# schwallergroup/matinvent

Measured on AMD Instinct MI355X. Metric: crystal structures/sec (1000-step reverse diffusion), higher is better.
Workload: dtype f32 via 2-plane fp16 split (3 fp16 MFMA terms, f32 accumulate)

## Files before the change

### matinvent_amd/csrc/edge_stage.hip

```cpp
#include <mutex>

#include <cstdio>
#include <cstdlib>
#include "net.h"
#include "gemm_split.h"
#define MI_LOOP_BARRIER() __builtin_amdgcn_s_barrier()
#define MI_RING_WAIT(w) asm volatile("s_waitcnt vmcnt(20)" : "+v"((w)[0][0]), "+v"((w)[0][1]), "+v"((w)[1][0]), "+v"((w)[1][1]))

namespace mi {

extern int g_edge2_train;
int g_edge2_fused = 1;

#if MI_PLANES_FP16

struct EdgeGemm2Args {
    Planes A;
    const u16* W2f;
    const float* b2;
    const float* dsc;
    const int* src;
    const int* rowptr;
    float* part;
    int E, N;
    const int* tab = nullptr;
    float* Z2 = nullptr;
    unsigned long long* clk;
};

constexpr int EG2_TAB = 2 + 128 + 128;
__global__ __launch_bounds__(128) void edge2_tables_kernel(const int* __restrict__ src, const int* __restrict__ rowptr, int E, int N, int* __restrict__ tab) {
    const int tile = blockIdx.x, tid = threadIdx.x, row0 = tile * 128;
    if (row0 >= E) return;
    const int nrows = E - row0 < 128 ? E - row0 : 128;
    const int node_first = src[row0];
    int* t = tab + (size_t)tile * EG2_TAB;
    const int r = row0 + tid, node = node_first + tid;
    t[2 + tid] = r < E ? src[r] - node_first : -1;
    t[130 + tid] = node < N ? tile - (rowptr[node] >> 7) : 0;
    if (tid == 0) {
        t[0] = node_first;
        t[1] = src[row0 + nrows - 1] - node_first + 1;
    }
}

constexpr int EG2B_STAGE = 2 * 128 * 64, EG2B_NST = 4;
constexpr int EG2B_LDS = EG2B_NST * EG2B_STAGE + 128 * 4 + 128 * 4;

template <int D, bool SAVE_Z = false>
__global__ __launch_bounds__(256) __attribute__((amdgpu_waves_per_eu(2, 2))) void edge_gemm2b_kernel(EdgeGemm2Args a) {
    constexpr int H = 512, KS = H / 16, KT = H / 32;
    extern __shared__ __attribute__((aligned(16))) unsigned char smem[];
    int* srcl = reinterpret_cast<int*>(smem + EG2B_NST * EG2B_STAGE);
    int* slotb = srcl + 128;
    const int tid = threadIdx.x, lane = tid & 63, wave = __builtin_amdgcn_readfirstlane(tid >> 6);
    const int l31 = lane & 31, kg = lane >> 5;
    const int id = blockIdx.x, slot = id >> 3, half = slot & 1, tile = (slot >> 1) * 8 + (id & 7);
    const int row0 = tile * 128;
    if (row0 >= a.E) return;
    const int nrows = a.E - row0 < 128 ? a.E - row0 : 128;
    int stamp_i = 0;
    auto stamp = [&]() {
        if (a.clk && tid == 0) a.clk[(size_t)(tile * 2 + half) * 8 + stamp_i] = __builtin_amdgcn_s_memtime();
        ++stamp_i;
    };
    stamp();
    if (a.clk && tid == 0) a.clk[(size_t)(tile * 2 + half) * 8 + 4] = __builtin_amdgcn_s_memrealtime();

    const int* tab = a.tab + (size_t)tile * EG2_TAB;
    int t_srcl = -1, t_slotb = 0;
    if (tid < 128) {
        t_srcl = tab[2 + tid];
        t_slotb = tab[130 + tid];
    }
    const int node_first = tab[0], cnt_tab = tab[1];

    const __amdgpu_buffer_rsrc_t rsa = uniform_rsrc(a.A.base + a.A.tile(tile, 0), a.A.KT * 24576);
    const int voffa = (lane >> 2) * 64 + (((lane & 3) ^ ((lane >> 4) & 3)) << 4);
    auto dma_tile = [&](int kt, int st) {
#pragma unroll
        for (int q = 0; q < 4; ++q) {
            const int piece = wave * 4 + q;
            __builtin_amdgcn_raw_ptr_buffer_load_lds(rsa, (__attribute__((address_space(3))) void*)(smem + st * EG2B_STAGE + piece * 1024), 16, voffa,
                                                     kt * 24576 + (piece >> 3) * 8192 + (piece & 7) * 1024, 0, 0);
        }
    };
    dma_tile(0, 0);
    dma_tile(1, 1);
    dma_tile(2, 2);

    int voffw[2];
#pragma unroll
    for (int t = 0; t < 2; ++t) voffw[t] = lane * 16 + ((8 * half + 2 * wave + t) * KS) * 2048;
    u32x4 ring[D][2][2];
    const u32x4 rsw_s = rsrc_words(a.W2f, H * H * 4);
    auto ring_load = [&](int ks, u32x4 (&w)[2][2]) {
        const int soff = __builtin_amdgcn_readfirstlane(ks * 2048);
#pragma unroll
        for (int t = 0; t < 2; ++t) {
            asm volatile("buffer_load_dwordx4 %0, %1, %2, %3 offen" : "=v"(w[t][0]) : "v"(voffw[t]), "s"(rsw_s), "s"(soff));
            asm volatile("buffer_load_dwordx4 %0, %1, %2, %3 offen offset:1024" : "=v"(w[t][1]) : "v"(voffw[t]), "s"(rsw_s), "s"(soff));
        }
    };
#pragma unroll
    for (int d = 0; d < D; ++d) ring_load(d, ring[d]);

    if (tid < 128) {
        srcl[tid] = t_srcl;
        slotb[tid] = t_slotb;
    }
    const float os = a.dsc[1] * (1.f / PL_SW), s_m2 = a.dsc[2], inv_m2 = a.dsc[3];

    f32x16 acc[4][2];
#pragma unroll
    for (int i = 0; i < 4; ++i)
#pragma unroll
        for (int j = 0; j < 2; ++j)
#pragma unroll
            for (int r = 0; r < 16; ++r) acc[i][j][r] = 0.f;
    const unsigned lds0 = (unsigned)(uintptr_t)(__attribute__((address_space(3))) unsigned char*)smem;
    unsigned rd_off[2];
#pragma unroll
    for (int s2 = 0; s2 < 2; ++s2) rd_off[s2] = lds0 + (unsigned)(l31 * 64 + (((2 * s2 + kg) ^ ((l31 >> 2) & 3)) * 16));
    auto read_a = [&](int st, int s2, f16x8 (&af)[4][2]) {
        const unsigned va = rd_off[s2] + (unsigned)st * EG2B_STAGE;
#define MI_RD128(dst, off) asm volatile("ds_read_b128 %0, %1 offset:%2" : "=v"(dst) : "v"(va), "n"(off))
        MI_RD128(af[0][0], 0 * 2048);        MI_RD128(af[0][1], 0 * 2048 + 8192);
        MI_RD128(af[1][0], 1 * 2048);        MI_RD128(af[1][1], 1 * 2048 + 8192);
        MI_RD128(af[2][0], 2 * 2048);        MI_RD128(af[2][1], 2 * 2048 + 8192);
        MI_RD128(af[3][0], 3 * 2048);        MI_RD128(af[3][1], 3 * 2048 + 8192);
#undef MI_RD128
    };
    auto mma = [&](const u32x4 (&w)[2][2], f16x8 (&af)[4][2]) {
#pragma unroll
        for (int ip = 0; ip < 2; ++ip) {
            if (ip == 0) asm volatile("s_waitcnt lgkmcnt(4)" : "+v"(af[0][0]), "+v"(af[0][1]), "+v"(af[1][0]), "+v"(af[1][1]));
            else asm volatile("s_waitcnt lgkmcnt(0)" : "+v"(af[2][0]), "+v"(af[2][1]), "+v"(af[3][0]), "+v"(af[3][1]));
#pragma unroll
            for (int term = MI_TERM0; term < 3; ++term)
#pragma unroll
                for (int i = 2 * ip; i < 2 * ip + 2; ++i)
#pragma unroll
                    for (int j = 0; j < 2; ++j)
                        acc[i][j] = __builtin_amdgcn_mfma_f32_32x32x16_f16(af[i][term == 0 ? 1 : 0], __builtin_bit_cast(f16x8, w[j][term == 1 ? 1 : 0]), acc[i][j], 0, 0, 0);
        }
    };
    static_assert(D == 4, "two k-tiles of ring per unrolled pair of iterations");
#pragma unroll 1
    for (int kt = 0; kt < KT; kt += 2) {
#pragma unroll
        for (int h2 = 0; h2 < 2; ++h2) {
            const int k = kt + h2;
            if (k == 0 || k >= KT - 3) asm volatile("s_waitcnt vmcnt(0)" ::: "memory");
            else asm volatile("s_waitcnt vmcnt(24)" ::: "memory");
            MI_LOOP_BARRIER();
            if (k == 0) stamp();
            if (k + 3 < KT) dma_tile(k + 3, (k + 3) & 3);
            f16x8 af[4][2];
#pragma unroll
            for (int s2 = 0; s2 < 2; ++s2) {
                read_a(k & 3, s2, af);
                MI_RING_WAIT(ring[2 * h2 + s2]);
                mma(ring[2 * h2 + s2], af);
                if (2 * k + s2 + D < KS) ring_load(2 * k + s2 + D, ring[2 * h2 + s2]);
                __builtin_amdgcn_sched_barrier(0);
            }
        }
    }
    stamp();

    if constexpr (SAVE_Z) {
        __syncthreads();
        float* stage = reinterpret_cast<float*>(smem) + wave * 1152;
#pragma unroll
        for (int i = 0; i < 4; ++i)
#pragma unroll
            for (int j = 0; j < 2; ++j) {
                const int rb = row0 + i * 32, cb = half * 256 + wave * 64 + j * 32;
#pragma unroll
                for (int r = 0; r < 16; ++r) stage[((r & 3) + 8 * (r >> 2) + 4 * kg) * 36 + l31] = acc[i][j][r] * os;
                __builtin_amdgcn_wave_barrier();
#pragma unroll
                for (int u = 0; u < 2; ++u) {
                    const int q = lane + 64 * u, rl = q >> 2, c8 = (q & 3) * 8;
                    const int row = rb + rl, col = cb + c8;
                    f32x4 z0 = *reinterpret_cast<const f32x4*>(stage + rl * 36 + c8);
                    f32x4 z1 = *reinterpret_cast<const f32x4*>(stage + rl * 36 + c8 + 4);
                    if (row < a.E) {
                        z0 += *reinterpret_cast<const f32x4*>(a.b2 + col);
                        z1 += *reinterpret_cast<const f32x4*>(a.b2 + col + 4);
                        float* d = a.Z2 + (size_t)row * H + col;
                        *reinterpret_cast<f32x4*>(d) = z0;
                        *reinterpret_cast<f32x4*>(d + 4) = z1;
                    }
                }
                __builtin_amdgcn_wave_barrier();
            }
    }

    const int cnt = nrows > 0 ? cnt_tab : 0;
    u16* sfr = reinterpret_cast<u16*>(smem);
    unsigned sat = 0;
    const int nlb = (cnt + 31) >> 5;
    __syncthreads();
    for (int f = tid; f < nlb * 8 * 64; f += 256) {
        const int ln = f & 63, fu = (f >> 6) & 1, frb = (f >> 7) & 3, fq = f >> 9;
        const int me = fq * 32 + (ln & 31), fkg = ln >> 5;
        u32x4 w;
#pragma unroll
        for (int i2 = 0; i2 < 4; ++i2) {
            const int ia = 2 * i2, ib = 2 * i2 + 1;
            const int ra = frb * 32 + 4 * fkg + 8 * (2 * fu + (ia >> 2)) + (ia & 3), rbb = frb * 32 + 4 * fkg + 8 * (2 * fu + (ib >> 2)) + (ib & 3);
            w[i2] = (srcl[ra] == me ? 0x3C00u : 0u) | (srcl[rbb] == me ? 0x3C000000u : 0u);
        }
        *reinterpret_cast<u32x4*>(sfr + (size_t)f * 8) = w;
    }
    __syncthreads();
#pragma unroll
    for (int j = 0; j < 2; ++j) {
        __builtin_amdgcn_sched_barrier(0);
        const int col = half * 256 + wave * 64 + j * 32 + l31;
        const float bcol = a.b2[col];
#pragma unroll 1
        for (int lb0 = 0; lb0 < nlb; lb0 += 2) {
            const bool two = lb0 + 1 < nlb;
            f32x16 ps[2];
#pragma unroll
            for (int q = 0; q < 2; ++q)
#pragma unroll
                for (int r = 0; r < 16; ++r) ps[q][r] = 0.f;
#pragma unroll
            for (int rb = 0; rb < 4; ++rb) {
                const f32x16 av = acc[rb][j];
#pragma unroll
                for (int u = 0; u < 2; ++u) {
                    f16x8 mh, ml;
#pragma unroll
                    for (int idx = 0; idx < 8; idx += 2) {
                        const float v0 = silu_fast(av[8 * u + idx] * os + bcol), v1 = silu_fast(av[8 * u + idx + 1] * os + bcol);
                        unsigned p[3];
                        pl_split_pair_acc(v0, v1, s_m2, p, sat);
                        const f16x2 h = __builtin_bit_cast(f16x2, p[0]), lo = __builtin_bit_cast(f16x2, p[1]);
                        mh[idx] = h[0]; mh[idx + 1] = h[1];
                        ml[idx] = lo[0]; ml[idx + 1] = lo[1];
                    }
#pragma unroll
                    for (int q = 0; q < 2; ++q) {
                        if (q == 1 && !two) break;
                        const f16x8 sf = *reinterpret_cast<const f16x8*>(sfr + (size_t)((((lb0 + q) * 4 + rb) * 2 + u) * 64 + lane) * 8);
                        ps[q] = __builtin_amdgcn_mfma_f32_32x32x16_f16(sf, ml, ps[q], 0, 0, 0);
                        ps[q] = __builtin_amdgcn_mfma_f32_32x32x16_f16(sf, mh, ps[q], 0, 0, 0);
                    }
                    __builtin_amdgcn_sched_barrier(0);
                }
            }
#pragma unroll
            for (int q = 0; q < 2; ++q)
#pragma unroll
                for (int r = 0; r < 16; ++r) {
                    const int loc = (lb0 + q) * 32 + (r & 3) + 8 * (r >> 2) + 4 * kg;
                    if (loc < cnt) a.part[((size_t)slotb[loc] * a.N + node_first + loc) * H + col] = ps[q][r] * inv_m2;
                }
        }
    }
    stamp();
    if (a.clk && tid == 0) a.clk[(size_t)(tile * 2 + half) * 8 + 5] = __builtin_amdgcn_s_memrealtime();
    sat_report(sat);
}

template <bool EXT, bool LEAN = false>
__global__ __launch_bounds__(256) __attribute__((amdgpu_waves_per_eu(2, 2))) void gemm_rt_kernel(Planes A, const u16* __restrict__ Wf, int M, int N, int K,
                                                                                                 PlanesEpilogue pe, unsigned long long* __restrict__ clk) {
    const int KS = K >> 4, KT = K >> 5;
    extern __shared__ __attribute__((aligned(16))) unsigned char smem[];
    M = pe.rows(M);
    const int tid = threadIdx.x, lane = tid & 63, wave = __builtin_amdgcn_readfirstlane(tid >> 6);
    int stamp_i = 0;
    auto stamp = [&]() {
        if (clk && tid == 0) clk[(size_t)blockIdx.x * 8 + stamp_i] = __builtin_amdgcn_s_memtime();
        ++stamp_i;
    };
    stamp();
    if (clk && tid == 0) clk[(size_t)blockIdx.x * 8 + 4] = __builtin_amdgcn_s_memrealtime();
    const int l31 = lane & 31, kg = lane >> 5;
    const int ncb = N >> 8;
    const int id = blockIdx.x, slot = id >> 3, cb = slot % ncb, tile = (slot / ncb) * 8 + (id & 7);
    const int row0 = tile * 128;
    if (row0 >= M) return;

    const __amdgpu_buffer_rsrc_t rsa = uniform_rsrc(A.base + A.tile(tile, 0), A.KT * 24576);
    const int voffa = (lane >> 2) * 64 + (((lane & 3) ^ ((lane >> 4) & 3)) << 4);
    auto dma_tile = [&](int kt, int st) {
#pragma unroll
        for (int q = 0; q < 4; ++q) {
            const int piece = wave * 4 + q;
            __builtin_amdgcn_raw_ptr_buffer_load_lds(rsa, (__attribute__((address_space(3))) void*)(smem + st * EG2B_STAGE + piece * 1024), 16, voffa,
                                                     kt * 24576 + (piece >> 3) * 8192 + (piece & 7) * 1024, 0, 0);
        }
    };
    dma_tile(0, 0);
    dma_tile(1, 1);
    dma_tile(2, 2);

    int voffw[2];
#pragma unroll
    for (int t = 0; t < 2; ++t) voffw[t] = lane * 16 + ((8 * cb + 2 * wave + t) * KS) * 2048;
    u32x4 ring[4][2][2];
    const u32x4 rsw_s = rsrc_words(Wf, N * K * 4);
    auto ring_load = [&](int ks, u32x4 (&w)[2][2]) {
        const int soff = __builtin_amdgcn_readfirstlane(ks * 2048);
#pragma unroll
        for (int t = 0; t < 2; ++t) {
            asm volatile("buffer_load_dwordx4 %0, %1, %2, %3 offen" : "=v"(w[t][0]) : "v"(voffw[t]), "s"(rsw_s), "s"(soff));
            asm volatile("buffer_load_dwordx4 %0, %1, %2, %3 offen offset:1024" : "=v"(w[t][1]) : "v"(voffw[t]), "s"(rsw_s), "s"(soff));
        }
    };
#pragma unroll
    for (int d = 0; d < 4; ++d) ring_load(d, ring[d]);

    f32x16 acc[4][2];
#pragma unroll
    for (int i = 0; i < 4; ++i)
#pragma unroll
        for (int j = 0; j < 2; ++j)
#pragma unroll
            for (int r = 0; r < 16; ++r) acc[i][j][r] = 0.f;
    const unsigned lds0 = (unsigned)(uintptr_t)(__attribute__((address_space(3))) unsigned char*)smem;
    unsigned rd_off[2];
#pragma unroll
    for (int s2 = 0; s2 < 2; ++s2) rd_off[s2] = lds0 + (unsigned)(l31 * 64 + (((2 * s2 + kg) ^ ((l31 >> 2) & 3)) * 16));
    auto read_a = [&](int st, int s2, f16x8 (&af)[4][2]) {
        const unsigned va = rd_off[s2] + (unsigned)st * EG2B_STAGE;
#define MI_RD128(dst, off) asm volatile("ds_read_b128 %0, %1 offset:%2" : "=v"(dst) : "v"(va), "n"(off))
        MI_RD128(af[0][0], 0 * 2048);        MI_RD128(af[0][1], 0 * 2048 + 8192);
        MI_RD128(af[1][0], 1 * 2048);        MI_RD128(af[1][1], 1 * 2048 + 8192);
        MI_RD128(af[2][0], 2 * 2048);        MI_RD128(af[2][1], 2 * 2048 + 8192);
        MI_RD128(af[3][0], 3 * 2048);        MI_RD128(af[3][1], 3 * 2048 + 8192);
#undef MI_RD128
    };
    auto mma = [&](const u32x4 (&w)[2][2], f16x8 (&af)[4][2]) {
#pragma unroll
        for (int ip = 0; ip < 2; ++ip) {
            if (ip == 0) asm volatile("s_waitcnt lgkmcnt(4)" : "+v"(af[0][0]), "+v"(af[0][1]), "+v"(af[1][0]), "+v"(af[1][1]));
            else asm volatile("s_waitcnt lgkmcnt(0)" : "+v"(af[2][0]), "+v"(af[2][1]), "+v"(af[3][0]), "+v"(af[3][1]));
#pragma unroll
            for (int term = MI_TERM0; term < 3; ++term)
#pragma unroll
                for (int i = 2 * ip; i < 2 * ip + 2; ++i)
#pragma unroll
                    for (int j = 0; j < 2; ++j)
                        if constexpr (LEAN)
                            acc[i][j] = __builtin_amdgcn_mfma_f32_32x32x16_f16(__builtin_bit_cast(f16x8, w[j][term == 1 ? 1 : 0]), af[i][term == 0 ? 1 : 0], acc[i][j], 0, 0, 0);
                        else
                            acc[i][j] = __builtin_amdgcn_mfma_f32_32x32x16_f16(af[i][term == 0 ? 1 : 0], __builtin_bit_cast(f16x8, w[j][term == 1 ? 1 : 0]), acc[i][j], 0, 0, 0);
        }
    };
#pragma unroll 1
    for (int kt = 0; kt < KT; kt += 2) {
#pragma unroll
        for (int h2 = 0; h2 < 2; ++h2) {
            const int k = kt + h2;
            if (k == 0 || k >= KT - 3) asm volatile("s_waitcnt vmcnt(0)" ::: "memory");
            else asm volatile("s_waitcnt vmcnt(24)" ::: "memory");
            MI_LOOP_BARRIER();
            if (k == 0) stamp();
            if (k + 3 < KT) dma_tile(k + 3, (k + 3) & 3);
            f16x8 af[4][2];
#pragma unroll
            for (int s2 = 0; s2 < 2; ++s2) {
                read_a(k & 3, s2, af);
                MI_RING_WAIT(ring[2 * h2 + s2]);
                mma(ring[2 * h2 + s2], af);
                if (2 * k + s2 + 4 < KS) ring_load(2 * k + s2 + 4, ring[2 * h2 + s2]);
                __builtin_amdgcn_sched_barrier(0);
            }
        }
    }
    __syncthreads();
    stamp();
    if constexpr (LEAN) planes_epilogue_lean<4, 2>(pe, acc, tile, cb * 256 + wave * 64, M, lane);
    else planes_epilogue_rows<4, 2, EXT>(pe, acc, row0, cb * 256 + wave * 64, M, N, lane, reinterpret_cast<float*>(smem) + wave * 1152);
    stamp();
    if (clk && tid == 0) clk[(size_t)blockIdx.x * 8 + 5] = __builtin_amdgcn_s_memrealtime();
}

__global__ void pack_frag_from_planes_kernel(Planes W, int N, int K, u16* __restrict__ dst) {
    const int KS = K / 16;
    const int64_t idx = (int64_t)blockIdx.x * blockDim.x + threadIdx.x;
    if (idx >= (int64_t)N * (K / 8)) return;
    const int r = (int)(idx / (K / 8)), ch = (int)(idx % (K / 8));
    const int ct = r >> 5, l31 = r & 31, ks = ch >> 1, kg = ch & 1;
#pragma unroll
    for (int pl = 0; pl < 2; ++pl)
        *reinterpret_cast<u32x4*>(dst + ((((size_t)ct * KS + ks) * 2 + pl) * 64 + kg * 32 + l31) * 8) = *reinterpret_cast<const u32x4*>(W.base + W.elem(r, ch * 8, pl));
}

int g_edge1_fused = 9;

__global__ void pack_frag_wff_pair_kernel(const float* __restrict__ W1, int edge_in, int H, int F, int Kh, u16* __restrict__ dst) {
    const int K = 2 * Kh, KS = K / 16, F3 = 3 * F;
    const int64_t idx = (int64_t)blockIdx.x * blockDim.x + threadIdx.x;
    if (idx >= (int64_t)H * (K / 8)) return;
    const int r = (int)(idx / (K / 8)), ch = (int)(idx % (K / 8));
    const int ct = r >> 5, l31 = r & 31, ks = ch >> 1, kg = ch & 1;
    float v[8];
#pragma unroll
    for (int i = 0; i < 8; ++i) {
        const int c = ch * 8 + i, blk = c >= Kh, cc = blk ? c - Kh : c;
        v[i] = cc < F3 ? W1[(size_t)r * edge_in + 2 * H + 9 + blk * F3 + cc] : 0.f;
    }
    u32x4 pk[2];
#pragma unroll
    for (int i = 0; i < 4; ++i) {
        unsigned p[3];
        pl_split_pair(v[2 * i], v[2 * i + 1], PL_SW, p);
        pk[0][i] = p[0];
        pk[1][i] = p[1];
    }
#pragma unroll
    for (int pl = 0; pl < 2; ++pl) *reinterpret_cast<u32x4*>(dst + ((((size_t)ct * KS + ks) * 2 + pl) * 64 + kg * 32 + l31) * 8) = pk[pl];
}

template <int D, bool WIDE>
__device__ __forceinline__ void edge_gemm1_body(const Planes& A, const u16* __restrict__ Wf, int M, int N, int K, PlanesEpilogue& pe, unsigned long long* clk) {
    extern __shared__ __attribute__((aligned(16))) unsigned char smem[];
    const int tid = threadIdx.x, lane = tid & 63, wave = __builtin_amdgcn_readfirstlane(tid >> 6);
    const int l31 = lane & 31, kg = lane >> 5;
    constexpr int MI = 4, NJ = 1;
    constexpr int WM = 4 / MI, WN = 4 / WM, WGC = 32 * NJ * WN;
    const int KT = K / 32, KS = K / 16, nq = N / WGC;
    const int wm = wave / WN, wn = wave % WN;
    const int id = blockIdx.x;
    float cps_local = 0.f;
    auto eval_scales = [&]() {
        if (pe.sc_pq) {
            float dsc[6];
            act_scales_eval(__uint_as_float(pe.sc_pq[0]), __uint_as_float(pe.sc_gmax[0]), pe.sc_wb, dsc);
            cps_local = dsc[0];
            if (id == 0 && tid < 6) {
                pe.sc_dsc[tid] = dsc[tid];
                if (pe.sc_dsc2) pe.sc_dsc2[tid] = dsc[tid];
            }
        }
    };
    eval_scales();
    if (pe.diag_C0 && id >= pe.diag_block0) {
        const float cps = cps_local != 0.f ? cps_local : pe.Cp.s();
        const int n0 = (id - pe.diag_block0) * 8, n1 = n0 + 8 < pe.diag_nodes ? n0 + 8 : pe.diag_nodes;
        const float* PQ = pe.ep.row_bias;
        const int ldpq = pe.ep.ld_row_bias;
        for (int f = 2 * tid; f < N; f += 512) {
            const float c0 = pe.diag_C0[f], c1 = pe.diag_C0[f + 1];
            for (int i = n0; i < n1; ++i) {
                const int e = pe.diag_e[i], g = pe.diag_node2graph[i];
                const float* G = pe.ep.row_bias3 + (size_t)g * pe.ep.ld_row_bias3;
                const float v0 = c0 + ((PQ[(size_t)i * ldpq + f] + PQ[(size_t)i * ldpq + N + f]) + G[f]);
                const float v1 = c1 + ((PQ[(size_t)i * ldpq + f + 1] + PQ[(size_t)i * ldpq + N + f + 1]) + G[f + 1]);
                if (pe.ep.pre_act) {
                    pe.ep.pre_act[(size_t)e * pe.ep.ld_pre + f] = v0;
                    pe.ep.pre_act[(size_t)e * pe.ep.ld_pre + f + 1] = v1;
                }
                unsigned p[3];
                pl_split_pair(silu_fast(v0), silu_fast(v1), cps, p);
#pragma unroll
                for (int k = 0; k < NPL; ++k) *reinterpret_cast<unsigned*>(pe.Cp.base + pe.Cp.elem(e, f, k)) = p[k];
            }
        }
        return;
    }
    const int slot = id >> 3, qt = slot % nq, tile = (slot / nq) * 8 + (id & 7);
    const int row0 = tile * 128;
    if (row0 >= M) return;
    int stamp_i = 0;
    auto stamp = [&]() {
        if (clk && tid == 0) clk[(size_t)(tile * nq + qt) * 8 + stamp_i] = __builtin_amdgcn_s_memtime();
        ++stamp_i;
    };
    stamp();

    const __amdgpu_buffer_rsrc_t rsa = uniform_rsrc(A.base + A.tile(tile, 0), A.KT * 24576);
    const int voffa = (lane >> 2) * 64 + (((lane & 3) ^ ((lane >> 4) & 3)) << 4);
    auto dma_tile = [&](int kt, int st) {
#pragma unroll
        for (int q = 0; q < 4; ++q) {
            const int piece = wave * 4 + q;
            __builtin_amdgcn_raw_ptr_buffer_load_lds(rsa, (__attribute__((address_space(3))) void*)(smem + st * EG2B_STAGE + piece * 1024), 16, voffa,
                                                     kt * 24576 + (piece >> 3) * 8192 + (piece & 7) * 1024, 0, 0);
        }
    };
    dma_tile(0, 0);
    dma_tile(1, 1);
    dma_tile(2, 2);
    const __amdgpu_buffer_rsrc_t rsw = uniform_rsrc(Wf, N * K * 4);
    int voffw[NJ];
#pragma unroll
    for (int t = 0; t < NJ; ++t) voffw[t] = lane * 16 + (((WN * qt + wn) * NJ + t) * KS) * 2048;
    u32x4 ring[D][NJ][2];
    const u32x4 rsw_s = rsrc_words(Wf, N * K * 4);
    auto ring_load = [&](int ks, u32x4 (&w)[NJ][2]) {
        const int soff = __builtin_amdgcn_readfirstlane(ks * 2048);
        asm volatile("buffer_load_dwordx4 %0, %1, %2, %3 offen" : "=v"(w[0][0]) : "v"(voffw[0]), "s"(rsw_s), "s"(soff));
        asm volatile("buffer_load_dwordx4 %0, %1, %2, %3 offen offset:1024" : "=v"(w[0][1]) : "v"(voffw[0]), "s"(rsw_s), "s"(soff));
    };
#pragma unroll
    for (int d = 0; d < D; ++d) ring_load(d, ring[d]);

    f32x16 acc[MI][NJ], accS[MI][NJ];
#pragma unroll
    for (int i = 0; i < MI; ++i)
#pragma unroll
        for (int j = 0; j < NJ; ++j)
#pragma unroll
            for (int r = 0; r < 16; ++r) acc[i][j][r] = 0.f;
    const unsigned lds0 = (unsigned)(uintptr_t)(__attribute__((address_space(3))) unsigned char*)smem;
    unsigned rd_off[2];
#pragma unroll
    for (int s2 = 0; s2 < 2; ++s2) rd_off[s2] = lds0 + (unsigned)(l31 * 64 + (((2 * s2 + kg) ^ ((l31 >> 2) & 3)) * 16));
    auto read_a = [&](int st, int s2, f16x8 (&af)[MI][2]) {
        const unsigned va = rd_off[s2] + (unsigned)st * EG2B_STAGE;
#define MI_RD128(dst, off) asm volatile("ds_read_b128 %0, %1 offset:%2" : "=v"(dst) : "v"(va), "n"(off))
        MI_RD128(af[0][0], 0 * 2048);        MI_RD128(af[0][1], 0 * 2048 + 8192);
        MI_RD128(af[1][0], 1 * 2048);        MI_RD128(af[1][1], 1 * 2048 + 8192);
        MI_RD128(af[2][0], 2 * 2048);        MI_RD128(af[2][1], 2 * 2048 + 8192);
        MI_RD128(af[3][0], 3 * 2048);        MI_RD128(af[3][1], 3 * 2048 + 8192);
#undef MI_RD128
    };
    auto mma = [&](u32x4 (&w)[NJ][2], f16x8 (&af)[MI][2]) {
        asm volatile("s_waitcnt vmcnt(14)" : "+v"(w[0][0]), "+v"(w[0][1]));
#pragma unroll
        for (int ip = 0; ip < 2; ++ip) {
            if (ip == 0) asm volatile("s_waitcnt lgkmcnt(4)" : "+v"(af[0][0]), "+v"(af[0][1]), "+v"(af[1][0]), "+v"(af[1][1]));
            else asm volatile("s_waitcnt lgkmcnt(0)" : "+v"(af[2][0]), "+v"(af[2][1]), "+v"(af[3][0]), "+v"(af[3][1]));
#pragma unroll
            for (int term = MI_TERM0; term < 3; ++term)
#pragma unroll
                for (int i = 2 * ip; i < 2 * ip + 2; ++i)
                    acc[i][0] = __builtin_amdgcn_mfma_f32_32x32x16_f16(af[i][term == 0 ? 1 : 0], __builtin_bit_cast(f16x8, w[0][term == 1 ? 1 : 0]), acc[i][0], 0, 0, 0);
        }
    };
    static_assert(D == 4, "two k-tiles of ring per unrolled pair of iterations");
    const int khalf = KT / 2;
#pragma unroll 1
    for (int kt = 0; kt < KT; kt += 2) {
#pragma unroll
        for (int h2 = 0; h2 < 2; ++h2) {
            const int k = kt + h2;
            if (k == khalf) {
#pragma unroll
                for (int i = 0; i < MI; ++i)
#pragma unroll
                    for (int j = 0; j < NJ; ++j) {
                        accS[i][j] = acc[i][j];
#pragma unroll
                        for (int r = 0; r < 16; ++r) acc[i][j][r] = 0.f;
                    }
            }
            if (k == 0 || k >= KT - 3) asm volatile("s_waitcnt vmcnt(0)" ::: "memory");
            else asm volatile("s_waitcnt vmcnt(16)" ::: "memory");
            MI_LOOP_BARRIER();
            if (k == 0) stamp();
            if (k + 3 < KT) dma_tile(k + 3, (k + 3) & 3);
            f16x8 af[MI][2];
#pragma unroll
            for (int s2 = 0; s2 < 2; ++s2) {
                read_a(k & 3, s2, af);
                mma(ring[2 * h2 + s2], af);
                if (2 * k + s2 + D < KS) ring_load(2 * k + s2 + D, ring[2 * h2 + s2]);
                __builtin_amdgcn_sched_barrier(0);
            }
        }
    }
    stamp();
    __syncthreads();
    planes_epilogue_pairs<MI, NJ, WIDE>(pe, accS, acc, row0 + wm * MI * 32, qt * WGC + wn * 32 * NJ, M, N, lane, reinterpret_cast<float*>(smem) + wave * 2304, cps_local);
    stamp();
}

template <int D, bool WIDE = true>
__global__ __launch_bounds__(256) __attribute__((amdgpu_waves_per_eu(2, 2))) void edge_gemm1b_kernel(Planes A, const u16* __restrict__ Wf, int M, int N, int K,
                                                                                                     PlanesEpilogue pe, unsigned long long* clk) {
    edge_gemm1_body<D, WIDE>(A, Wf, M, N, K, pe, clk);
}

unsigned long long* g_edge1_clk = nullptr;

__global__ void empty_boundary_kernel() {}

int edge_gemm1(mi_net* net, const Planes& A, int layer, int M, PlanesEpilogue pe, hipStream_t s) {
    if (g_ablate_skip & 2) return MI_OK;
    if (g_ablate_skip & 32) hipLaunchKernelGGL(empty_boundary_kernel, dim3(1), dim3(64), 0, s);
    static std::once_flag once;
    static hipError_t attr_err = hipSuccess;
    std::call_once(once, [] {
        attr_err = hipFuncSetAttribute((const void*)edge_gemm1b_kernel<4>, hipFuncAttributeMaxDynamicSharedMemorySize, EG2B_LDS);
        if (attr_err == hipSuccess) attr_err = hipFuncSetAttribute((const void*)edge_gemm1b_kernel<4, false>, hipFuncAttributeMaxDynamicSharedMemorySize, EG2B_LDS);
    });
    MI_HIP(attr_err);
    const int H = net->H, K = 2 * net->Kh;
    count_mfma(M, H, K, MI_PLANES_TERMS);
    pe.out_scale = 1.f / (A.scale * PL_SW);
    int nblk = (H / 128) * ((cdiv(M, 128) + 7) / 8 * 8);
    if (pe.diag_C0) {
        pe.diag_block0 = nblk;
        nblk += cdiv(pe.diag_nodes, 8);
    }
    const u16* Wf = net->Wffc + (size_t)layer * ((size_t)H * K * 2);
    if (pe.pair_wide) hipLaunchKernelGGL((edge_gemm1b_kernel<4>), dim3(nblk), dim3(256), EG2B_LDS, s, A, Wf, M, H, K, pe, g_edge1_clk);
    else hipLaunchKernelGGL((edge_gemm1b_kernel<4, false>), dim3(nblk), dim3(256), EG2B_LDS, s, A, Wf, M, H, K, pe, g_edge1_clk);
    MI_KERNEL_CHECK();
    return MI_OK;
}

bool edge_gemm1_supported(const mi_net* net, int64_t M) {
    if (!(net->H % 128 == 0 && net->Wffc != nullptr && (2 * net->Kh) % 64 == 0) || g_edge1_fused == 0) return false;
    if (g_edge1_fused != 9) return true;
    return (int64_t)(net->H / 128) * ((cdiv(M, 128) + 7) / 8 * 8) > g_planes_lat_max_blocks;
}

int edge_gemm1_pack(mi_net* net, int l, const float* W1, hipStream_t s) {
    const int H = net->H, K = 2 * net->Kh;
    hipLaunchKernelGGL(pack_frag_wff_pair_kernel, dim3(cdiv((int64_t)H * (K / 8), 256)), dim3(256), 0, s, W1, net->edge_in, H, net->F, net->Kh,
                       net->Wffc + (size_t)l * ((size_t)H * K * 2));
    MI_KERNEL_CHECK();
    return MI_OK;
}

unsigned long long* g_edge2_clk = nullptr;

int edge_gemm2(mi_net* net, mi_batch* b, int layer, hipStream_t s, float* Z2) {
    if (g_ablate_skip & 4) return MI_OK;
    if (g_ablate_skip & 32) hipLaunchKernelGGL(empty_boundary_kernel, dim3(1), dim3(64), 0, s);
    static std::once_flag once;
    static hipError_t attr_err = hipSuccess;
    std::call_once(once, [] {
        attr_err = hipFuncSetAttribute((const void*)edge_gemm2b_kernel<4>, hipFuncAttributeMaxDynamicSharedMemorySize, EG2B_LDS);
        if (attr_err == hipSuccess) attr_err = hipFuncSetAttribute((const void*)edge_gemm2b_kernel<4, true>, hipFuncAttributeMaxDynamicSharedMemorySize, EG2B_LDS);
    });
    MI_HIP(attr_err);
    const int H = net->H;
    count_mfma(b->E, H, H, MI_PLANES_TERMS);
    EdgeGemm2Args a;
    a.A = make_planes(b->m1_cur ? b->m1_cur : b->M1pl, H, PL_S_ACT, b->dsc);
    a.W2f = net->Wnc + (size_t)layer * node_chain_pack_elems(H) + (size_t)5 * H * H * 2;
    a.b2 = net->p("csp_layer_" + std::to_string(layer) + ".edge_mlp.2.bias");
    a.dsc = b->dsc;
    a.src = b->src;
    a.rowptr = b->rowptr;
    a.part = b->part;
    a.E = (int)b->E;
    a.N = b->N;
    {
        const int tiles_cap = cdiv(b->E_cap, 128);
        if (!b->e2_tab) MI_TRY(dev_alloc(b, &b->e2_tab, (size_t)tiles_cap * EG2_TAB));
        if (b->e2_tab_epoch != b->graph_epoch) {
            hipLaunchKernelGGL(edge2_tables_kernel, dim3(cdiv(b->E, 128)), dim3(128), 0, s, b->src, b->rowptr, (int)b->E, b->N, b->e2_tab);
            MI_KERNEL_CHECK();
            b->e2_tab_epoch = b->graph_epoch;
        }
        a.tab = b->e2_tab;
    }
    a.Z2 = Z2;
    a.clk = g_edge2_clk;
    if (Z2) {
        hipLaunchKernelGGL((edge_gemm2b_kernel<4, true>), dim3(2 * ((cdiv(b->E, 128) + 7) / 8 * 8)), dim3(256), EG2B_LDS, s, a);
        MI_KERNEL_CHECK();
        return MI_OK;
    }
    hipLaunchKernelGGL((edge_gemm2b_kernel<4>), dim3(2 * ((cdiv(b->E, 128) + 7) / 8 * 8)), dim3(256), EG2B_LDS, s, a);
    MI_KERNEL_CHECK();
    return MI_OK;
}

bool edge_gemm2_supported(const mi_net* net) { return g_edge2_fused && net->H == 512 && net->Wnc != nullptr; }

unsigned long long* g_rt_clk = nullptr;
int g_rt_clk_ext = -1;
int g_rt_lean = 1;
int g_rt_clk_skip = 0;

int gemm_rt(const Planes& A, const u16* Wfrag, int M, int N, int K, const PlanesEpilogue& pe, bool ext, hipStream_t s) {
    static std::once_flag once;
    static hipError_t attr_err = hipSuccess;
    std::call_once(once, [] {
        attr_err = hipFuncSetAttribute((const void*)gemm_rt_kernel<false>, hipFuncAttributeMaxDynamicSharedMemorySize, EG2B_NST * EG2B_STAGE);
        if (attr_err == hipSuccess) attr_err = hipFuncSetAttribute((const void*)gemm_rt_kernel<true>, hipFuncAttributeMaxDynamicSharedMemorySize, EG2B_NST * EG2B_STAGE);
        if (attr_err == hipSuccess) attr_err = hipFuncSetAttribute((const void*)gemm_rt_kernel<false, true>, hipFuncAttributeMaxDynamicSharedMemorySize, EG2B_NST * EG2B_STAGE);
        if (const char* e = getenv("MI_RT_LEAN")) g_rt_lean = atoi(e) & 3;
    });
    MI_HIP(attr_err);
    MI_CHECK(Wfrag && (N & 255) == 0 && (K & 63) == 0 && K >= 128 && A.KT >= K / 32, MI_EINVAL, "gemm_rt: N % 256, K % 64, K >= 128 and a fragment-order W operand");
    if (M <= 0) return MI_OK;
    count_mfma(M, N, K, MI_PLANES_TERMS);
    const dim3 grid((N >> 8) * ((cdiv(M, 128) + 7) / 8 * 8));
    static const bool trace = getenv("MI_RT_TRACE") != nullptr;
    if (trace)
        fprintf(stderr, "gemm_rt M=%d N=%d K=%d ext=%d act=%d bias=%d rb=%d%d%d pre_add=%d pre_act=%d res=%d res_pl=%d os=%g res2=%d res2_pl=%d rows2=%d post_mul=%d C=%d Cp=%d absmax=%d\n", M, N, K,
                (int)ext, pe.ep.act, !!pe.ep.bias, !!pe.ep.row_bias, !!pe.ep.row_bias2, !!pe.ep.row_bias3, !!pe.ep.pre_add, !!pe.ep.pre_act, !!pe.ep.residual, !!pe.res_pl.base,
                (double)pe.ep.out_scale, !!pe.residual2, !!pe.res2_pl.base, !!pe.res2_rows, !!pe.post_mul, !!pe.C, !!pe.Cp.base, !!pe.absmax);
    unsigned long long* clk = nullptr;
    if (g_rt_clk && (g_rt_clk_ext < 0 || g_rt_clk_ext == (int)ext)) {
        if (g_rt_clk_skip > 0) {
            --g_rt_clk_skip;
        } else {
            clk = g_rt_clk;
            if (g_rt_clk_ext >= 0) g_rt_clk = nullptr;
        }
    }
    if (g_rt_lean && planes_epilogue_is_lean(pe)) hipLaunchKernelGGL((gemm_rt_kernel<false, true>), grid, dim3(256), EG2B_NST * EG2B_STAGE, s, A, Wfrag, M, N, K, pe, clk);
    else if (ext) hipLaunchKernelGGL(gemm_rt_kernel<true>, grid, dim3(256), EG2B_NST * EG2B_STAGE, s, A, Wfrag, M, N, K, pe, clk);
    else hipLaunchKernelGGL(gemm_rt_kernel<false>, grid, dim3(256), EG2B_NST * EG2B_STAGE, s, A, Wfrag, M, N, K, pe, clk);
    MI_KERNEL_CHECK();
    return MI_OK;
}

size_t frag_elems(int N, int K) { return (size_t)N * K * 2; }

int pack_frag_from_planes(const Planes& W, int N, int K, u16* dst, hipStream_t s) {
    MI_CHECK((N & 31) == 0 && (K & 15) == 0, MI_EINVAL, "pack_frag_from_planes: N % 32, K % 16");
    hipLaunchKernelGGL(pack_frag_from_planes_kernel, dim3((unsigned)cdiv((int64_t)N * (K / 8), 256)), dim3(256), 0, s, W, N, K, dst);
    MI_KERNEL_CHECK();
    return MI_OK;
}

#else

int gemm_rt(const Planes&, const u16*, int, int, int, const PlanesEpilogue&, bool, hipStream_t) { return MI_ESTATE; }
size_t frag_elems(int N, int K) { return (size_t)N * K * 2; }
int pack_frag_from_planes(const Planes&, int, int, u16*, hipStream_t) { return MI_ESTATE; }

int edge_gemm2(mi_net*, mi_batch*, int, hipStream_t, float*) { return MI_ESTATE; }
bool edge_gemm2_supported(const mi_net*) { return false; }
int edge_gemm1(mi_net*, const Planes&, int, int, PlanesEpilogue, hipStream_t) { return MI_ESTATE; }
bool edge_gemm1_supported(const mi_net*, int64_t) { return false; }
int edge_gemm1_pack(mi_net*, int, const float*, hipStream_t) { return MI_OK; }
int g_edge1_fused = 0;

#endif

}

extern "C" int mi_debug_set_rt_lean(int on) {
#if MI_PLANES_FP16
    const int was = mi::g_rt_lean;
    mi::g_rt_lean = on & 3;
    return was;
#else
    (void)on;
    return 0;
#endif
}

extern "C" int mi_debug_rt_clock(void* dev_buffer, int ext, int skip) {
#if MI_PLANES_FP16
    mi::g_rt_clk = (unsigned long long*)dev_buffer;
    mi::g_rt_clk_ext = ext;
    mi::g_rt_clk_skip = skip;
#else
    (void)dev_buffer; (void)ext; (void)skip;
#endif
    return MI_OK;
}

extern "C" int mi_debug_edge2_clock(void* dev_buffer) {
#if MI_PLANES_FP16
    mi::g_edge2_clk = (unsigned long long*)dev_buffer;
#endif
    return MI_OK;
}

extern "C" int mi_debug_edge1_clock(void* dev_buffer) {
#if MI_PLANES_FP16
    mi::g_edge1_clk = (unsigned long long*)dev_buffer;
#endif
    return MI_OK;
}

extern "C" int mi_debug_set_edge2_fused(int on) {
    const int was = (mi::g_edge2_fused == 1 && !mi::g_edge2_train) ? 4 : mi::g_edge2_fused;
    mi::g_edge2_fused = on == 4 ? 1 : on;
    mi::g_edge2_train = on == 1;
    return was;
}

extern "C" int mi_debug_set_edge_fused(int) { return 0; }

extern "C" int mi_debug_set_edge1_fused(int on) {
    const int was = mi::g_edge1_fused;
    mi::g_edge1_fused = on;
    return was;
}
```

Baseline: 55.82.

## Fold self-edge diagonal work into GEMM tiles instead of extra tail blocks

Removes the separate tail blocks that computed self-edge (diagonal) activations after the GEMM grid. Each GEMM tile block now takes a share of diagonal nodes, loads their bias rows with vectorized loads while its DMA and weight prefetch are in flight, and computes the SiLU plus plane split itself. The first result is held in registers and stored after the epilogue. This is meant to cut the tail imbalance and extra block scheduling, at the cost of more register pressure and extra global traffic inside the GEMM prologue.

Measured after the change: 55.85, median of 2. Within noise of the previous version (+0.1%).

```diff
diff --git a/matinvent_amd/csrc/edge_stage.hip b/matinvent_amd/csrc/edge_stage.hip
--- a/matinvent_amd/csrc/edge_stage.hip
+++ b/matinvent_amd/csrc/edge_stage.hip
@@ -4,6 +4,7 @@
 #include <cstdlib>
 #include "net.h"
 #include "gemm_split.h"
+#include "self_edge_share.h"
 #define MI_LOOP_BARRIER() __builtin_amdgcn_s_barrier()
 #define MI_RING_WAIT(w) asm volatile("s_waitcnt vmcnt(20)" : "+v"((w)[0][0]), "+v"((w)[0][1]), "+v"((w)[1][0]), "+v"((w)[1][1]))
 
@@ -443,33 +444,17 @@
             }
         }
     };
-    eval_scales();
-    if (pe.diag_C0 && id >= pe.diag_block0) {
-        const float cps = cps_local != 0.f ? cps_local : pe.Cp.s();
-        const int n0 = (id - pe.diag_block0) * 8, n1 = n0 + 8 < pe.diag_nodes ? n0 + 8 : pe.diag_nodes;
-        const float* PQ = pe.ep.row_bias;
-        const int ldpq = pe.ep.ld_row_bias;
-        for (int f = 2 * tid; f < N; f += 512) {
-            const float c0 = pe.diag_C0[f], c1 = pe.diag_C0[f + 1];
-            for (int i = n0; i < n1; ++i) {
-                const int e = pe.diag_e[i], g = pe.diag_node2graph[i];
-                const float* G = pe.ep.row_bias3 + (size_t)g * pe.ep.ld_row_bias3;
-                const float v0 = c0 + ((PQ[(size_t)i * ldpq + f] + PQ[(size_t)i * ldpq + N + f]) + G[f]);
-                const float v1 = c1 + ((PQ[(size_t)i * ldpq + f + 1] + PQ[(size_t)i * ldpq + N + f + 1]) + G[f + 1]);
-                if (pe.ep.pre_act) {
-                    pe.ep.pre_act[(size_t)e * pe.ep.ld_pre + f] = v0;
-                    pe.ep.pre_act[(size_t)e * pe.ep.ld_pre + f + 1] = v1;
-                }
-                unsigned p[3];
-                pl_split_pair(silu_fast(v0), silu_fast(v1), cps, p);
-#pragma unroll
-                for (int k = 0; k < NPL; ++k) *reinterpret_cast<unsigned*>(pe.Cp.base + pe.Cp.elem(e, f, k)) = p[k];
-            }
-        }
-        return;
-    }
     const int slot = id >> 3, qt = slot % nq, tile = (slot / nq) * 8 + (id & 7);
     const int row0 = tile * 128;
+    int se_n0 = 0, se_n1 = 0;
+    if (pe.diag_C0) self_edge_share(tile, M, pe.diag_nodes, se_n0, se_n1);
+    const int se_i0 = se_n0 + (tid >> 4), se_col = qt * WGC + (tid & 15) * 8;
+    int se_e0 = 0, se_g0 = 0;
+    if (se_i0 < se_n1) {
+        se_e0 = pe.diag_e[se_i0];
+        se_g0 = pe.diag_node2graph[se_i0];
+    }
+    eval_scales();
     if (row0 >= M) return;
     int stamp_i = 0;
     auto stamp = [&]() {
@@ -477,6 +462,31 @@
         ++stamp_i;
     };
     stamp();
+
+    auto se_frow = [&](const float* base, int r, int ld, int c) -> const float* {
+        if constexpr (WIDE) return base + (size_t)r * ld + c;
+        else return reinterpret_cast<const float*>(reinterpret_cast<const char*>(base) + ((unsigned)r * ((unsigned)ld * 4u) + (unsigned)c * 4u));
+    };
+    auto se_load = [&](int i, int g, f32x4 (&r)[6]) {
+        const float* pi = se_frow(pe.ep.row_bias, i, pe.ep.ld_row_bias, se_col);
+        const float* pj = se_frow(pe.ep.row_bias, i, pe.ep.ld_row_bias, N + se_col);
+        const float* gg = se_frow(pe.ep.row_bias3, g, pe.ep.ld_row_bias3, se_col);
+        r[0] = *reinterpret_cast<const f32x4*>(pi);
+        r[1] = *reinterpret_cast<const f32x4*>(pi + 4);
+        r[2] = *reinterpret_cast<const f32x4*>(pj);
+        r[3] = *reinterpret_cast<const f32x4*>(pj + 4);
+        r[4] = *reinterpret_cast<const f32x4*>(gg);
+        r[5] = *reinterpret_cast<const f32x4*>(gg + 4);
+    };
+    f32x4 se_c0[2] = {}, se_r[6] = {};
+    const float se_cps = cps_local != 0.f ? cps_local : se_n0 < se_n1 ? pe.Cp.s() : 0.f;
+    __builtin_amdgcn_s_waitcnt(0x0f70);
+    if (se_i0 < se_n1) {
+        se_c0[0] = *reinterpret_cast<const f32x4*>(pe.diag_C0 + se_col);
+        se_c0[1] = *reinterpret_cast<const f32x4*>(pe.diag_C0 + se_col + 4);
+        se_load(se_i0, se_g0, se_r);
+    }
+    __builtin_amdgcn_sched_barrier(0);
 
     const __amdgpu_buffer_rsrc_t rsa = uniform_rsrc(A.base + A.tile(tile, 0), A.KT * 24576);
     const int voffa = (lane >> 2) * 64 + (((lane & 3) ^ ((lane >> 4) & 3)) << 4);
@@ -504,6 +514,51 @@
     };
 #pragma unroll
     for (int d = 0; d < D; ++d) ring_load(d, ring[d]);
+
+    u32x4 se_o[3] = {};
+    auto se_store = [&](int e, const u32x4 (&o)[3]) {
+        const unsigned tile_stride_b = ((unsigned)pe.Cp.KT * 12288u + 2048u) * 2u;
+#pragma unroll
+        for (int pl = 0; pl < NPL; ++pl) {
+            u16* dst;
+            if constexpr (WIDE) dst = pe.Cp.base + pe.Cp.elem(e, se_col, pl);
+            else dst = reinterpret_cast<u16*>(reinterpret_cast<char*>(pe.Cp.base + pl * 4096) +
+                                              (((unsigned)e >> 7) * tile_stride_b + (((unsigned)e & 127u) << 6) + ((unsigned)(se_col >> 5) * 24576u + ((unsigned)se_col & 31u) * 2u)));
+            *reinterpret_cast<u32x4*>(dst) = o[pl];
+        }
+    };
+    if (se_n0 < se_n1) {
+        for (int i = se_i0; i < se_n1; i += 16) {
+            int e = se_e0;
+            if (i != se_i0) {
+                e = pe.diag_e[i];
+                se_load(i, pe.diag_node2graph[i], se_r);
+            }
+            float v[8];
+#pragma unroll
+            for (int k = 0; k < 8; ++k) v[k] = se_c0[k >> 2][k & 3] + ((se_r[k >> 2][k & 3] + se_r[2 + (k >> 2)][k & 3]) + se_r[4 + (k >> 2)][k & 3]);
+            if (pe.ep.pre_act) {
+                float* d = const_cast<float*>(se_frow(pe.ep.pre_act, e, pe.ep.ld_pre, se_col));
+                *reinterpret_cast<f32x4*>(d) = f32x4{v[0], v[1], v[2], v[3]};
+                *reinterpret_cast<f32x4*>(d + 4) = f32x4{v[4], v[5], v[6], v[7]};
+            }
+            u32x4 o[3];
+#pragma unroll
+            for (int k = 0; k < 4; ++k) {
+                unsigned p[3];
+                pl_split_pair(silu_fast(v[2 * k]), silu_fast(v[2 * k + 1]), se_cps, p);
+                o[0][k] = p[0];
+                o[1][k] = p[1];
+                o[2][k] = p[2];
+            }
+            if (i == se_i0) {
+#pragma unroll
+                for (int pl = 0; pl < 3; ++pl) se_o[pl] = o[pl];
+            } else {
+                se_store(e, o);
+            }
+        }
+    }
 
     f32x16 acc[MI][NJ], accS[MI][NJ];
 #pragma unroll
@@ -573,6 +628,7 @@
     stamp();
     __syncthreads();
     planes_epilogue_pairs<MI, NJ, WIDE>(pe, accS, acc, row0 + wm * MI * 32, qt * WGC + wn * 32 * NJ, M, N, lane, reinterpret_cast<float*>(smem) + wave * 2304, cps_local);
+    if (se_i0 < se_n1) se_store(se_e0, se_o);
     stamp();
 }
 
@@ -599,11 +655,7 @@
     const int H = net->H, K = 2 * net->Kh;
     count_mfma(M, H, K, MI_PLANES_TERMS);
     pe.out_scale = 1.f / (A.scale * PL_SW);
-    int nblk = (H / 128) * ((cdiv(M, 128) + 7) / 8 * 8);
-    if (pe.diag_C0) {
-        pe.diag_block0 = nblk;
-        nblk += cdiv(pe.diag_nodes, 8);
-    }
+    const int nblk = (H / 128) * ((cdiv(M, 128) + 7) / 8 * 8);
     const u16* Wf = net->Wffc + (size_t)layer * ((size_t)H * K * 2);
     if (pe.pair_wide) hipLaunchKernelGGL((edge_gemm1b_kernel<4>), dim3(nblk), dim3(256), EG2B_LDS, s, A, Wf, M, H, K, pe, g_edge1_clk);
     else hipLaunchKernelGGL((edge_gemm1b_kernel<4, false>), dim3(nblk), dim3(256), EG2B_LDS, s, A, Wf, M, H, K, pe, g_edge1_clk);
diff --git a/matinvent_amd/csrc/self_edge_share.h b/matinvent_amd/csrc/self_edge_share.h
--- /dev/null
+++ b/matinvent_amd/csrc/self_edge_share.h
@@ -0,0 +1,22 @@
+#pragma once
+
+#if defined(__HIPCC__) || defined(__CUDACC__)
+#define MI_SE_HD __host__ __device__
+#else
+#define MI_SE_HD
+#endif
+
+namespace mi {
+
+MI_SE_HD inline void self_edge_share(int tile, int M, int N, int& n0, int& n1) {
+    const int T = (M + 127) / 128;
+    if (tile < 0 || tile >= T) {
+        n0 = n1 = 0;
+        return;
+    }
+    const int npt = (N + T - 1) / T;
+    n0 = tile * npt < N ? tile * npt : N;
+    n1 = n0 + npt < N ? n0 + npt : N;
+}
+
+}
```
